# facebookresearch/FRL-Distributed-ML-Scaffold

Hardware: NVIDIA H100
Metric: samples/sec (whole box) on synthetic 2-task Problem (higher is better)
Workload: dtype bf16

## Files before the change

### frl-distributed-ml-scaffold_b200/_native.py

```python
import ctypes as C
import os
import subprocess
from typing import Optional, Sequence

import torch

_HERE = os.path.dirname(os.path.abspath(__file__))
CSRC_DIR = os.path.join(_HERE, "csrc")
LIB_PATH = os.path.join(CSRC_DIR, "libfrl_b200.so")

F32, BF16, U8, I64 = 0, 1, 2, 3
LOSS_MSE, LOSS_CE, LOSS_CE_PROB = 0, 1, 2
FP8_E4M3, FP8_E5M2 = 0, 1
FP8_DTYPE = {FP8_E4M3: torch.float8_e4m3fn, FP8_E5M2: torch.float8_e5m2}
MAX_TASKS = 8

_DTYPE_CODE = {torch.float32: F32, torch.bfloat16: BF16, torch.uint8: U8, torch.bool: U8,
               torch.int64: I64}


class NativeLibraryError(RuntimeError):
    pass


# ... 19 lines not shown
    "frl_launch_count": (C.c_uint64, []),
    "frl_launch_count_reset": (None, []),
    "frl_device_sm_count": (_i, []),
    "frl_device_arch": (_i, []),
    "frl_sgd_momentum": (_i, [_vp, _vp, _vp, _vp, _i64, _d, _d, _d, _d, _d, _vp, _vp, _i, _i, _vp]),
    "frl_adam": (_i, [_vp, _vp, _vp, _vp, _vp, _vp, _i64, _d, _d, _d, _d, _d, _i64, _d, _vp, _vp, _i, _vp]),
    "frl_rmsprop": (_i, [_vp, _vp, _vp, _vp, _vp, _i64, _d, _d, _d, _d, _d, _d, _vp, _vp, _i, _vp]),
    "frl_mt_tile_elems": (_i64, []),
    "frl_flatten_grads": (_i, [_vp, _vp, _vp, _i64, _vp, _i, _d, _vp]),
    "frl_sgd_momentum_mt": (_i, [_vp, _vp, _vp, _vp, _vp, _vp, _i64, _d, _d, _d, _d, _d, _vp, _vp, _i, _vp]),
    "frl_adam_mt": (_i, [_vp, _vp, _vp, _vp, _vp, _vp, _vp, _vp, _i64, _d, _d, _d, _d, _d, _i64, _d, _vp, _vp, _vp]),
    "frl_rmsprop_mt": (_i, [_vp, _vp, _vp, _vp, _vp, _vp, _vp, _i64, _d, _d, _d, _d, _d, _d, _vp, _vp, _vp]),
    "frl_layerwise_scratch_bytes": (_i64, [_i64, _i64]),
    "frl_lars_mt": (_i, [_vp, _vp, _vp, _vp, _vp, _vp, _i64, _i64, _vp, _vp, _vp, _d, _d, _d, _d, _vp, _vp, _i, _vp]),
    "frl_lamb_mt": (_i, [_vp, _vp, _vp, _vp, _vp, _vp, _vp, _i64, _i64, _vp, _vp, _vp, _d, _d, _d, _d, _d, _i64,
                         _d, _vp, _vp, _vp]),
    "frl_grad_accumulate_mt": (_i, [_vp, _vp, _vp, _vp, _i64, _d, _i, _vp, _vp]),
    "frl_weight_ema": (_i, [_vp, _vp, _i64, _d, _vp]),
    "frl_reduce_scratch_bytes": (_i64, []),
    "frl_grad_sumsq_clip": (_i, [_vp, _i64, _i, _f, _f, _vp, _vp, _vp]),
    "frl_criteria_scratch_bytes": (_i64, [_i]),
    "frl_criteria_forward": (_i, [C.POINTER(TaskDesc), _i, _vp, _vp, _vp, _vp, _vp, _vp, _vp]),
    "frl_criteria_backward": (_i, [C.POINTER(TaskDesc), _i, _vp, _vp, _vp, _vp]),
    "frl_preproc_affine": (_i, [_vp, _i, _vp, _i, _i64, _i64, _i64, _vp, _vp, _vp]),
    "frl_cast_scale": (_i, [_vp, _i, _vp, _i, _i64, _f, _vp]),
    "frl_augment_images": (_i, [_vp, _i64, _i, _i, _i, _vp, C.c_uint64, _i, _i, _d, _d, _d, _d, _d, _i, _i,
                                _vp, _vp, _vp, _i, _i, _i, _vp, _vp]),
    "frl_augment_mix_images": (_i, [_vp, _i64, _i, _i, _i, _vp, C.c_uint64, _i, _i, _d, _d, _d, _d, _d, _i, _i,
                                    _vp, _vp, _vp, _i, _i, _i, _vp, _i, _f, _i, _i, _i, _i, _vp]),
    "frl_mix_targets": (_i, [_vp, _i, _i64, _i64, _i, _f, _vp, _vp]),
    "frl_colsum_scratch_bytes": (_i64, [_i64, _i64]),
    "frl_colsum": (_i, [_vp, _i, _i64, _i64, _vp, _i, _i, _vp, _vp]),
    "frl_drelu_colsum": (_i, [_vp, _vp, _vp, _i, _i64, _i64, _vp, _i, _i, _vp, _vp]),
    "frl_gather_rows": (_i, [_vp, _i64, _vp, _vp, _i64, _i64, _i, _vp]),
    "frl_gather_rows_tma": (_i, [_vp, _i64, _vp, _vp, _i64, _i64, _i, _vp]),
    "frl_gather_window_rows": (_i, [_vp, _vp, _i, _vp, _vp, _i64, _i64, _vp]),
    "frl_gather_lines": (_i, [_vp, _i64, _i64, _vp, _i64, _vp, _vp, _i64, _i64, _i, _i, _vp]),
    "frl_gather_pool_create": (_vp, [_i]),
    "frl_gather_pool_destroy": (None, [_vp]),
    "frl_gather_pool_threads": (_i, [_vp]),
    "frl_gather_pool_submit": (_i64, [_vp, _vp, _i64, _vp, _vp, _i64, _i64]),
    "frl_gather_pool_submit_f32_to_bf16": (_i64, [_vp, _vp, _i64, _vp, _vp, _i64, _i64]),
    "frl_gather_pool_wait": (_i, [_vp, _i64]),
    "frl_nvls_sgd": (_i, [_vp, _vp, _vp, _vp, _i64, _i, _i, _vp, _i, _vp, _i, _d, _d, _d, _d, _d, _vp, _i, _i, _i, _vp]),
    "frl_nvls_adam": (_i, [_vp, _vp, _vp, _vp, _vp, _vp, _i64, _i, _i, _vp, _i, _vp, _i, _d, _d, _d, _d, _d,
                           _i64, _d, _vp, _i, _i, _vp]),
# ... 196 lines not shown

def criteria_scratch_bytes(n_tasks: int) -> int:
    return int(lib().frl_criteria_scratch_bytes(n_tasks))


def make_task_array(descs: Sequence[TaskDesc]):
    arr = (TaskDesc * len(descs))()
    for i, d in enumerate(descs):
        arr[i] = d
    return arr


def criteria_forward(task_array, n_tasks, losses, aux, lse, sink, nan_flag, scratch) -> None:
    _check(lib().frl_criteria_forward(task_array, n_tasks, _ptr(losses), _ptr(aux), _ptr(lse),
                                      _ptr(sink), _ptr(nan_flag), _ptr(scratch), _stream()),
           "frl_criteria_forward")


def criteria_backward(task_array, n_tasks, grad_losses, aux, lse) -> None:
    _check(lib().frl_criteria_backward(task_array, n_tasks, _ptr(grad_losses), _ptr(aux),
                                       _ptr(lse), _stream()), "frl_criteria_backward")



def preproc_affine(src, dst, *, inner=1, channels=1, scale=None, bias=None) -> None:
    n = src.numel()
    assert dst.numel() == n and src.is_contiguous() and dst.is_contiguous()
    _check(lib().frl_preproc_affine(_ptr(src), dtype_code(src.dtype), _ptr(dst),
                                    dtype_code(dst.dtype), n, inner, channels, _ptr(scale),
                                    _ptr(bias), _stream()), "frl_preproc_affine")


AUG_RRC, AUG_PAD_CROP, AUG_CENTER_RESIZE, AUG_CENTER_CROP = 0, 1, 2, 3


MIX_MIXUP, MIX_CUTMIX = 1, 2


def _augment_args(src, idx, dst, seed, epoch, mode, scale_range, ratio_range, eval_crop, pad, flip, scale, bias,
                  params_out):
    B, Cc, H, W = src.shape
    assert src.dtype == torch.uint8 and src.is_contiguous() and dst.is_contiguous()
    assert dst.dim() == 4 and tuple(dst.shape[:2]) == (B, Cc)
    assert idx.dtype == torch.int64 and idx.is_contiguous() and idx.numel() == B
    assert params_out is None or (params_out.dtype == torch.int32 and params_out.is_contiguous()
                                  and tuple(params_out.shape) == (B, 5))
# ... 219 lines not shown
```

### frl-distributed-ml-scaffold_b200/arena_linear.py

```python
import os
import types
from collections import Counter
from typing import List, Optional

import torch
import torch.nn as nn
import torch.nn.functional as F

from . import _native
from .types import Precision

KERNELS = _native

FP8_MULTIPLE = 16


def fp8_site_qualifies(uses_lp: bool, in_features: int, out_features: int) -> bool:
    return bool(uses_lp) and in_features % FP8_MULTIPLE == 0 and out_features % FP8_MULTIPLE == 0


def fp8_call_qualifies(x: torch.Tensor) -> bool:
    if x.dim() == 0 or x.shape[-1] == 0 or x.dtype not in (torch.bfloat16, torch.float32):
        return False
    m = x.numel() // x.shape[-1]
# ... 106 lines not shown
            y2 = saved[-1].reshape(-1, dz.shape[1])
            if in_step:
                dz_relu = torch.empty_like(dz)
                KERNELS.drelu_colsum(dz, y2, dz_relu, pipe.arena.grad_view(site.bslot),
                                     accumulate=not site.bstate.first_touch(pipe.step_id))
                dz, db_written = dz_relu, True
            else:
                dz = torch.ops.aten.threshold_backward(dz, y2, 0)
        need_dx = ctx.needs_input_grad[0]
        gemms = (_Fp8Gemms if ctx.fp8 else _DenseGemms)(saved, dz, need_dx)
        dx = gemms.dx().view(ctx.x_shape) if need_dx else None
        if in_step:
            site.weight_grad(pipe, gemms)
            if ctx.has_bias and not db_written and site.bslot is not None:
                KERNELS.colsum(dz.contiguous(), pipe.arena.grad_view(site.bslot),
                               accumulate=not site.bstate.first_touch(pipe.step_id))
            site.backward_done(pipe)
            return dx, None, None, None, None, None
        dw = gemms.dw(gemms.dzt) if ctx.needs_input_grad[1] else None
        db = dz.sum(0) if (ctx.has_bias and ctx.needs_input_grad[2]) else None
        return dx, dw, db, None, None, None


class _ArenaMultiHeadFn(torch.autograd.Function):

    @staticmethod
    def forward(ctx, x, site, *params):
        ctx.site = site
        ctx.save_for_backward(x)
        ctx.n_heads = len(params) // 2
        return tuple(F.linear(x, params[2 * i], params[2 * i + 1]) for i in range(ctx.n_heads))

    @staticmethod
    @torch.autograd.function.once_differentiable
    def backward(ctx, *dys):
        (x,) = ctx.saved_tensors
        site = ctx.site
        pipe = site.pipeline
        dy = torch.cat(dys, dim=1)
        dx = dy.matmul(site.weight_cat()) if ctx.needs_input_grad[0] else None
        none = (None,) * (2 * ctx.n_heads)
        if pipe is not None and pipe.step_open:
            gw = site.grad_weight_cat()
            if site.heads[0].wstate.first_touch(pipe.step_id):
                torch.mm(dy.t(), x, out=gw)
            else:
                gw.addmm_(dy.t(), x)
            for h in site.heads[1:]:
                h.wstate.first_touch(pipe.step_id)
            gb = site.grad_bias_cat()
            if gb is not None:
                first = site.heads[0].bstate.first_touch(pipe.step_id)
                for h in site.heads[1:]:
                    h.bstate.first_touch(pipe.step_id)
                KERNELS.colsum(dy, gb, accumulate=not first)
            else:
                for h, dyi in zip(site.heads, dys):
                    KERNELS.colsum(dyi.contiguous(), pipe.arena.grad_view(h.bslot),
                                   accumulate=not h.bstate.first_touch(pipe.step_id))
            for h in site.heads:
                h.backward_done(pipe)
            return (dx, None) + none
# ... 252 lines not shown
```

### frl-distributed-ml-scaffold_b200/criteria.py

```python
from abc import ABC, abstractmethod
from typing import Dict, List, Optional, Sequence, Tuple

import numpy as np
import torch
import torch.nn as nn
import torch.nn.functional as F
import torch.nn.modules.loss as L

from . import _native
from .types import LossType

KERNELS = _native



class MaskedLoss(L._Loss):

    def __init__(self, loss_layer, reduction: str = "mean") -> None:
        super().__init__(reduction=reduction)
        self.loss_layer = loss_layer

    def forward(self, *inputs) -> torch.Tensor:
        output, target, mask = inputs
        assert not target.requires_grad
# ... 160 lines not shown
    @staticmethod
    def forward(ctx, plan: _Plan, _unused, *outputs):
        outs = [o.contiguous() for o in outputs[:plan.n]]
        dev = outs[0].device
        losses = torch.empty(1 + plan.n, dtype=torch.float32, device=dev)
        aux = torch.empty(plan.n, dtype=torch.float32, device=dev)
        n_lse = sum(o.shape[0] * (2 if tp.kind == _native.LOSS_CE_PROB else 1)
                    for o, tp in zip(outs, plan.tasks) if tp.kind != _native.LOSS_MSE)
        lse = torch.empty(max(n_lse, 1), dtype=torch.float32, device=dev)
        arr, keep = _descs(plan, outs, None)
        KERNELS.criteria_forward(arr, plan.n, losses, aux, lse, plan.sink, plan.nan_flag,
                                 _scratch_for(dev, plan.n))
        ctx.plan = plan
        ctx.save_for_backward(aux, lse, *outs)
        ctx.set_materialize_grads(True)
        return losses

    @staticmethod
    @torch.autograd.function.once_differentiable
    def backward(ctx, grad_losses):
        plan = ctx.plan
        aux, lse, *outs = ctx.saved_tensors
        gl = grad_losses.contiguous().float()
        douts = [torch.empty_like(o) for o in outs]
        arr, keep = _descs(plan, outs, douts)
        KERNELS.criteria_backward(arr, plan.n, gl, aux, lse)
        return (None, None, *douts)


_path_logged = set()


def _log_path_once(modules, fused: bool) -> None:
    key = (tuple(type(m).__name__ for m in modules), fused)
    if key not in _path_logged:
        _path_logged.add(key)
        import logging
        logging.getLogger(__name__).info(
            "criterion path for loss modules %s: %s", list(key[0]),
            "fused kernels (frl_criteria_forward / _backward, one launch each)" if fused else
            "composed torch ops — outside the fused kernels' domain (MSE / CrossEntropy with mean "
            "reduction, optionally inside MaskedLoss; not class-weighted CrossEntropy or per-position "
            "probability targets)")


def fused_task_losses(modules, outputs, targets, weights=None, sink=None, nan_flag=None
                      ) -> Optional[torch.Tensor]:
    if not outputs or not outputs[0].is_cuda:
        return None
    plan = _plan_for(modules, outputs, targets, weights)
# ... 169 lines not shown
```

### frl-distributed-ml-scaffold_b200/csrc/criteria.cu

```cuda
#include "frl_common.cuh"

namespace frl {

constexpr int kCThreads = 256;
constexpr int kCWarps = kCThreads / 32;
constexpr int kCMaxBlocksPerTask = 528;
constexpr int kCVecPerLane = 8;
constexpr int kCRowChunk = 32 * 4 * kCVecPerLane;

struct CritParams {
    frl_task_desc t[FRL_MAX_TASKS];
    int nblk[FRL_MAX_TASKS];
    int blk_start[FRL_MAX_TASKS];
    int part_off[FRL_MAX_TASKS];
    int64_t lse_off[FRL_MAX_TASKS];
    int n_tasks;
    int total_blocks;
};

struct CritScratchHeader {
    unsigned int ticket;
    unsigned int _pad[3];
};
static inline int64_t crit_scratch_bytes(int T) {
    return static_cast<int64_t>(sizeof(CritScratchHeader)) +
           3ll * T * kCMaxBlocksPerTask * static_cast<int64_t>(sizeof(float));
}

template <typename T> __device__ __forceinline__ float ldf(const void* base, int64_t i);
template <> __device__ __forceinline__ float ldf<float>(const void* base, int64_t i) {
    return __ldg(static_cast<const float*>(base) + i);
}
template <> __device__ __forceinline__ float ldf<__nv_bfloat16>(const void* base, int64_t i) {
    return __bfloat162float(__ldg(static_cast<const __nv_bfloat16*>(base) + i));
}
__device__ __forceinline__ float ld_any(const void* base, int dtype, int64_t i) {
    return dtype == FRL_F32 ? ldf<float>(base, i) : ldf<__nv_bfloat16>(base, i);
}
// ... 18 lines not shown
    *reinterpret_cast<f32x4*>(static_cast<float*>(base) + e) = v;
}
template <> __device__ __forceinline__ void st4<__nv_bfloat16>(void* base, int64_t e, const f32x4& v) {
    *reinterpret_cast<bf16x4*>(static_cast<__nv_bfloat16*>(base) + e) =
        bf16x4{pack_bf16(v.x, v.y), pack_bf16(v.z, v.w)};
}

template <typename T> struct Raw4;
template <> struct Raw4<float> { f32x4 v; };
template <> struct Raw4<__nv_bfloat16> { bf16x4 v; };
__device__ __forceinline__ Raw4<float> ldraw4(const float* base, int64_t e) {
    return Raw4<float>{*reinterpret_cast<const f32x4*>(base + e)};
}
__device__ __forceinline__ Raw4<__nv_bfloat16> ldraw4(const __nv_bfloat16* base, int64_t e) {
    return Raw4<__nv_bfloat16>{*reinterpret_cast<const bf16x4*>(base + e)};
}
__device__ __forceinline__ f32x4 cvt4(const Raw4<float>& r) { return r.v; }
__device__ __forceinline__ f32x4 cvt4(const Raw4<__nv_bfloat16>& r) {
    return f32x4{bf16lo(r.v.a), bf16hi(r.v.a), bf16lo(r.v.b), bf16hi(r.v.b)};
}
__device__ __forceinline__ void fill_neg_inf(Raw4<float>& r) { r.v = f32x4{-INFINITY, -INFINITY, -INFINITY, -INFINITY}; }
__device__ __forceinline__ void fill_neg_inf(Raw4<__nv_bfloat16>& r) { r.v = bf16x4{0xff80ff80u, 0xff80ff80u}; }

__device__ __forceinline__ bool vec_ok(const frl_task_desc& t) {
    const int esz = t.out_dtype == FRL_F32 ? 4 : 2;
    return (t.cols % 4 == 0) && ((reinterpret_cast<uintptr_t>(t.out) % (4 * esz)) == 0) &&
           (t.dout == nullptr || (reinterpret_cast<uintptr_t>(t.dout) % (4 * esz)) == 0);
}

template <typename OT>
__device__ __forceinline__ void mse_partial(const frl_task_desc& t, int blk, int nblk,
                                            float& sum, float& nsel) {
    const int64_t n = t.rows * t.cols;
    const int64_t stride = static_cast<int64_t>(nblk) * kCThreads;
    float s = 0.f, c = 0.f;
    for (int64_t e = static_cast<int64_t>(blk) * kCThreads + threadIdx.x; e < n; e += stride) {
        if (t.mask && t.mask[e / t.mask_inner] == 0) continue;
        const float d = ldf<OT>(t.out, e) - ld_any(t.tgt, t.tgt_dtype, e);
        s = fmaf(d, d, s);
        c += 1.f;
    }
    sum = s;
    nsel = c;
}

__device__ __forceinline__ float soft_w(const frl_task_desc& t, bool prob, int64_t r0, int64_t c, int64_t y,
                                       float keep, float eps_c) {
    if (prob) return fmaf(keep, ld_any(t.tgt, t.tgt_dtype, r0 + c), eps_c);
    return (c == y ? keep : 0.f) + eps_c;
}

template <typename OT, bool SOFT>
__device__ __forceinline__ void ce_partial(const frl_task_desc& t, int blk, int nblk, float* lse_out,
                                           float& sum, float& nsel, float& nvalid) {
    const int lane = threadIdx.x & 31, warp = threadIdx.x >> 5;
    const int64_t C = t.cols;
    const bool vec = vec_ok(t);
    const int64_t* labels = static_cast<const int64_t*>(t.tgt);
    const bool prob = SOFT && t.kind == FRL_LOSS_CE_PROB;
// ... 20 lines not shown
                m = fmaxf(fmaxf(m, fmaxf(v.x, v.y)), fmaxf(v.z, v.w));
            }
            m = warp_max(m);
#pragma unroll
            for (int j = 0; j < kCVecPerLane; ++j) {
                if (lane * 4 + j * 128 < C) {
                    const f32x4 v = cvt4(q[j]);
                    has_nan |= (v.x != v.x) | (v.y != v.y) | (v.z != v.z) | (v.w != v.w);
                    se += expf(v.x - m) + expf(v.y - m) + expf(v.z - m) + expf(v.w - m);
                    if (soft) {
                        const int64_t c = lane * 4 + j * 128;
                        const float w0 = soft_w(t, prob, r0, c, ys, keep, eps_c);
                        const float w1 = soft_w(t, prob, r0, c + 1, ys, keep, eps_c);
                        const float w2 = soft_w(t, prob, r0, c + 2, ys, keep, eps_c);
                        const float w3 = soft_w(t, prob, r0, c + 3, ys, keep, eps_c);
                        aw += w0 * (m - v.x) + w1 * (m - v.y) + w2 * (m - v.z) + w3 * (m - v.w);
                        sw += (w0 + w1) + (w2 + w3);
                    }
                }
            }
        } else if (vec) {
            float mr = -INFINITY, sr = 0.f;
            for (int64_t cb = 0; cb < C; cb += kCRowChunk) {
                f32x4 v[kCVecPerLane];
#pragma unroll
                for (int j = 0; j < kCVecPerLane; ++j) {
                    const int64_t c = cb + lane * 4 + j * 128;
                    v[j] = c < C ? ld4<OT>(t.out, r0 + c) : f32x4{-INFINITY, -INFINITY, -INFINITY, -INFINITY};
                }
                float ml = -INFINITY;
#pragma unroll
                for (int j = 0; j < kCVecPerLane; ++j)
                    ml = fmaxf(fmaxf(ml, fmaxf(v[j].x, v[j].y)), fmaxf(v[j].z, v[j].w));
                const float mn = fmaxf(mr, ml);
                float add = 0.f;
                if (soft && mr != -INFINITY) aw = fmaf(sw, mn - mr, aw);
#pragma unroll
                for (int j = 0; j < kCVecPerLane; ++j) {
                    if (cb + lane * 4 + j * 128 < C) {
                        has_nan |= (v[j].x != v[j].x) | (v[j].y != v[j].y) | (v[j].z != v[j].z) | (v[j].w != v[j].w);
                        add += expf(v[j].x - mn) + expf(v[j].y - mn) + expf(v[j].z - mn) + expf(v[j].w - mn);
                        if (soft) {
                            const int64_t c = cb + lane * 4 + j * 128;
                            const float w0 = soft_w(t, prob, r0, c, ys, keep, eps_c);
                            const float w1 = soft_w(t, prob, r0, c + 1, ys, keep, eps_c);
                            const float w2 = soft_w(t, prob, r0, c + 2, ys, keep, eps_c);
                            const float w3 = soft_w(t, prob, r0, c + 3, ys, keep, eps_c);
                            aw += w0 * (mn - v[j].x) + w1 * (mn - v[j].y) + w2 * (mn - v[j].z) + w3 * (mn - v[j].w);
                            sw += (w0 + w1) + (w2 + w3);
                        }
                    }
                }
                sr = (mn == -INFINITY) ? 0.f : fmaf(sr, expf(mr - mn), add);
                mr = mn;
            }
            m = warp_max(mr);
            se = (mr == -INFINITY) ? 0.f : sr * expf(mr - m);
            if (soft && mr != -INFINITY) aw = fmaf(sw, m - mr, aw);

        } else {
            for (int64_t c = lane; c < C; c += 32) m = fmaxf(m, ldf<OT>(t.out, r0 + c));
            m = warp_max(m);
            for (int64_t c = lane; c < C; c += 32) {
                const float x = ldf<OT>(t.out, r0 + c);
                has_nan |= (x != x);
                se += expf(x - m);
                if (soft) {
                    const float w = soft_w(t, prob, r0, c, ys, keep, eps_c);
                    aw = fmaf(w, m - x, aw);
                    sw += w;
                }
// ... 22 lines not shown
                    s_sel += 1.f;
                    if (ys != static_cast<int64_t>(t.ignore_index)) {
                        s_valid += 1.f;
                        s_loss += (ys >= 0 && ys < C && !has_nan) ? fmaf(sw, logf(se), aw)
                                                                 : __int_as_float(0x7fc00000);
                    }
                }
            } else if (sel) {
                s_sel += 1.f;
                const int64_t y = labels[row];
                if (y != static_cast<int64_t>(t.ignore_index)) {
                    s_valid += 1.f;
                    s_loss += (y >= 0 && y < C) ? (lse - ldf<OT>(t.out, r0 + y))
                                                : __int_as_float(0x7fc00000);
                }
            }
        }
    }
    sum = s_loss;
    nsel = s_sel;
    nvalid = s_valid;
}

template <bool SOFT>
__global__ void __launch_bounds__(kCThreads, 5)
criteria_fwd_kernel(const __grid_constant__ CritParams P, float* __restrict__ losses,
                    float* __restrict__ aux, float* __restrict__ lse,
                    float* __restrict__ sink, int32_t* __restrict__ nan_flag,
                    CritScratchHeader* __restrict__ hdr) {
    __shared__ float smem[32];
    __shared__ bool is_last;
    int ti = 0;
#pragma unroll
    for (int i = 1; i < FRL_MAX_TASKS; ++i)
        if (i < P.n_tasks && static_cast<int>(blockIdx.x) >= P.blk_start[i]) ti = i;
    const int blk = static_cast<int>(blockIdx.x) - P.blk_start[ti];
    const frl_task_desc& t = P.t[ti];
    const int npart = P.n_tasks * kCMaxBlocksPerTask;
    float* part_sum = reinterpret_cast<float*>(hdr + 1);
    float* part_sel = part_sum + npart;
    float* part_valid = part_sel + npart;

    float s = 0.f, nsel = 0.f, nvalid = 0.f;
    if (t.kind == FRL_LOSS_MSE) {
        if (t.out_dtype == FRL_F32) mse_partial<float>(t, blk, P.nblk[ti], s, nsel);
        else                        mse_partial<__nv_bfloat16>(t, blk, P.nblk[ti], s, nsel);
        nvalid = nsel;
    } else {
        float* lse_t = lse + P.lse_off[ti];
        if (t.out_dtype == FRL_F32) ce_partial<float, SOFT>(t, blk, P.nblk[ti], lse_t, s, nsel, nvalid);
        else                        ce_partial<__nv_bfloat16, SOFT>(t, blk, P.nblk[ti], lse_t, s, nsel, nvalid);
    }
    s = block_sum(s, smem);
    nsel = block_sum(nsel, smem);
    nvalid = block_sum(nvalid, smem);
    if (threadIdx.x == 0) {
        const int slot = P.part_off[ti] + blk;
        part_sum[slot] = s;
        part_sel[slot] = nsel;
        part_valid[slot] = nvalid;
        __threadfence();
        is_last = (atomicAdd(&hdr->ticket, 1u) == static_cast<unsigned int>(P.total_blocks - 1));
    }
    __syncthreads();
    if (!is_last) return;
    __threadfence();

    __shared__ double dsm[kCWarps][3];
    const int lane = threadIdx.x & 31, warp = threadIdx.x >> 5;
    float total = 0.f;
    for (int i = 0; i < P.n_tasks; ++i) {
        double ds = 0.0, dsel = 0.0, dvalid = 0.0;
        for (int b = threadIdx.x; b < P.nblk[i]; b += kCThreads) {
            ds += static_cast<double>(__ldcg(part_sum + P.part_off[i] + b));
// ... 18 lines not shown
            if (q.mask != nullptr && dsel == 0.0) {
                if (q.kind == FRL_LOSS_MSE)     Li = 0.f;
                else if (SOFT && q.kind == FRL_LOSS_CE_PROB) Li = q.label_smoothing * logf(static_cast<float>(q.cols));
                else if (q.ignore_index == 0)   Li = __int_as_float(0x7fc00000);
                else                            Li = logf(static_cast<float>(q.cols));
            } else {
                Li = static_cast<float>(ds / dvalid);
            }
            Li *= q.weight;
            aux[i] = dvalid > 0.0 ? static_cast<float>(1.0 / dvalid) : 0.f;
            losses[1 + i] = Li;
            if (sink) sink[1 + i] = Li;
            total += Li;
        }
    }
    if (threadIdx.x == 0) {
        losses[0] = total;
        if (sink) sink[0] = total;
        if (nan_flag && (total != total)) *nan_flag = 1;
        hdr->ticket = 0;
    }
}

template <typename OT>
__device__ __forceinline__ void mse_bwd(const frl_task_desc& t, int blk, int nblk, float coef) {
    const int64_t n = t.rows * t.cols;
    const int64_t stride = static_cast<int64_t>(nblk) * kCThreads;
    for (int64_t e = static_cast<int64_t>(blk) * kCThreads + threadIdx.x; e < n; e += stride) {
        float d = 0.f;
        if (!(t.mask && t.mask[e / t.mask_inner] == 0))
            d = (ldf<OT>(t.out, e) - ld_any(t.tgt, t.tgt_dtype, e)) * coef;
        stf<OT>(t.dout, e, d);
    }
}

template <typename OT, bool SOFT>
__device__ __forceinline__ void ce_bwd(const frl_task_desc& t, int blk, int nblk, const float* lse,
                                       float coef) {
    const int lane = threadIdx.x & 31, warp = threadIdx.x >> 5;
    const int64_t C = t.cols;
    const bool vec = vec_ok(t);
    const int64_t* labels = static_cast<const int64_t*>(t.tgt);
    const bool prob = SOFT && t.kind == FRL_LOSS_CE_PROB;
    const bool soft = SOFT && (prob || t.label_smoothing != 0.f);
    const float keep = 1.f - t.label_smoothing, eps_c = t.label_smoothing / static_cast<float>(C);
    for (int64_t row = static_cast<int64_t>(blk) * kCWarps + warp; row < t.rows;
         row += static_cast<int64_t>(nblk) * kCWarps) {
        const int64_t r0 = row * C;
        const int64_t y = prob ? -1 : labels[row];
        const bool use = ((t.mask == nullptr) || (t.mask[row] != 0)) &&
                         (prob || y != static_cast<int64_t>(t.ignore_index));
        const float k = use ? coef : 0.f;
        const float l = lse[row];
        if (soft) {
            const float sq = prob ? lse[t.rows + row] : 1.f;
            if (vec) {
                for (int64_t cb = 0; cb < C; cb += kCRowChunk) {
                    f32x4 v[kCVecPerLane];
#pragma unroll
                    for (int j = 0; j < kCVecPerLane; ++j) {
                        const int64_t c = cb + lane * 4 + j * 128;
                        if (c < C) v[j] = ld4<OT>(t.out, r0 + c);
                    }
#pragma unroll
                    for (int j = 0; j < kCVecPerLane; ++j) {
                        const int64_t c = cb + lane * 4 + j * 128;
                        if (c >= C) break;
                        f32x4 q = v[j];
                        q.x = (expf(q.x - l) * sq - soft_w(t, prob, r0, c + 0, y, keep, eps_c)) * k;
                        q.y = (expf(q.y - l) * sq - soft_w(t, prob, r0, c + 1, y, keep, eps_c)) * k;
                        q.z = (expf(q.z - l) * sq - soft_w(t, prob, r0, c + 2, y, keep, eps_c)) * k;
                        q.w = (expf(q.w - l) * sq - soft_w(t, prob, r0, c + 3, y, keep, eps_c)) * k;
                        if (!use) q = f32x4{0.f, 0.f, 0.f, 0.f};
                        st4<OT>(t.dout, r0 + c, q);
                    }
                }
            } else {
                for (int64_t c = lane; c < C; c += 32) {
                    const float x = ldf<OT>(t.out, r0 + c);
                    stf<OT>(t.dout, r0 + c,
                            use ? (expf(x - l) * sq - soft_w(t, prob, r0, c, y, keep, eps_c)) * k : 0.f);
                }
            }
        } else if (vec) {
            for (int64_t cb = 0; cb < C; cb += kCRowChunk) {
                f32x4 v[kCVecPerLane];
#pragma unroll
                for (int j = 0; j < kCVecPerLane; ++j) {
                    const int64_t c = cb + lane * 4 + j * 128;
                    if (c < C) v[j] = ld4<OT>(t.out, r0 + c);
                }
#pragma unroll
                for (int j = 0; j < kCVecPerLane; ++j) {
                    const int64_t c = cb + lane * 4 + j * 128;
                    if (c >= C) break;
                    f32x4 q = v[j];
                    q.x = (expf(q.x - l) - (c + 0 == y ? 1.f : 0.f)) * k;
                    q.y = (expf(q.y - l) - (c + 1 == y ? 1.f : 0.f)) * k;
                    q.z = (expf(q.z - l) - (c + 2 == y ? 1.f : 0.f)) * k;
                    q.w = (expf(q.w - l) - (c + 3 == y ? 1.f : 0.f)) * k;
                    if (!use) q = f32x4{0.f, 0.f, 0.f, 0.f};
                    st4<OT>(t.dout, r0 + c, q);
                }
            }
        } else {
            for (int64_t c = lane; c < C; c += 32) {
                const float x = ldf<OT>(t.out, r0 + c);
                stf<OT>(t.dout, r0 + c, use ? (expf(x - l) - (c == y ? 1.f : 0.f)) * k : 0.f);
            }
        }
    }
}

template <bool SOFT>
__global__ void __launch_bounds__(kCThreads, 5)
criteria_bwd_kernel(const __grid_constant__ CritParams P, const float* __restrict__ gl,
                    const float* __restrict__ aux, const float* __restrict__ lse) {
    int ti = 0;
#pragma unroll
    for (int i = 1; i < FRL_MAX_TASKS; ++i)
        if (i < P.n_tasks && static_cast<int>(blockIdx.x) >= P.blk_start[i]) ti = i;
    const int blk = static_cast<int>(blockIdx.x) - P.blk_start[ti];
    const frl_task_desc& t = P.t[ti];
    const float scale = (__ldg(gl) + __ldg(gl + 1 + ti)) * t.weight * __ldg(aux + ti);
    if (t.kind == FRL_LOSS_MSE) {
        const float coef = 2.f * scale;
        if (t.out_dtype == FRL_F32) mse_bwd<float>(t, blk, P.nblk[ti], coef);
        else                        mse_bwd<__nv_bfloat16>(t, blk, P.nblk[ti], coef);
    } else {
        const float* lse_t = lse + P.lse_off[ti];
        if (t.out_dtype == FRL_F32) ce_bwd<float, SOFT>(t, blk, P.nblk[ti], lse_t, scale);
        else                        ce_bwd<__nv_bfloat16, SOFT>(t, blk, P.nblk[ti], lse_t, scale);
    }
}

static int build_params(const frl_task_desc* tasks, int T, bool backward, CritParams& P, int& max_blk,
                        bool& soft, const char* name) {
    FRL_REQUIRE(tasks != nullptr && T >= 1, FRL_E_ARG, "%s: no tasks", name);
    FRL_REQUIRE(T <= FRL_MAX_TASKS, FRL_E_TOO_MANY, "%s: at most %d tasks", name, FRL_MAX_TASKS);
    int off = 0;
    int64_t lse_off = 0;
    max_blk = 1;
    soft = false;
    P.n_tasks = T;
    for (int i = 0; i < T; ++i) {
        const frl_task_desc& t = tasks[i];
        FRL_REQUIRE(t.kind == FRL_LOSS_MSE || t.kind == FRL_LOSS_CE || t.kind == FRL_LOSS_CE_PROB, FRL_E_ARG,
                    "%s: task %d kind", name, i);
        FRL_REQUIRE(t.label_smoothing >= 0.f && t.label_smoothing <= 1.f, FRL_E_ARG,
                    "%s: task %d label_smoothing must be in [0, 1], got %g", name, i, t.label_smoothing);
        FRL_REQUIRE(t.kind != FRL_LOSS_MSE || t.label_smoothing == 0.f, FRL_E_ARG,
                    "%s: task %d label_smoothing on an MSE task", name, i);
        FRL_REQUIRE(t.out_dtype == FRL_F32 || t.out_dtype == FRL_BF16, FRL_E_DTYPE, "%s: task %d out dtype", name, i);
        FRL_REQUIRE(t.rows >= 0 && t.cols >= 1, FRL_E_ARG, "%s: task %d shape", name, i);
        FRL_REQUIRE(t.rows == 0 || (t.out && t.tgt), FRL_E_ARG, "%s: task %d null out/tgt", name, i);
        FRL_REQUIRE(!backward || t.rows == 0 || t.dout, FRL_E_ARG, "%s: task %d null dout", name, i);
        if (t.kind == FRL_LOSS_MSE) {
            FRL_REQUIRE(t.tgt_dtype == FRL_F32 || t.tgt_dtype == FRL_BF16, FRL_E_DTYPE, "%s: task %d tgt dtype", name, i);
            FRL_REQUIRE(!t.mask || t.mask_inner >= 1, FRL_E_ARG, "%s: task %d mask_inner", name, i);
        } else if (t.kind == FRL_LOSS_CE_PROB) {
            FRL_REQUIRE(t.tgt_dtype == FRL_F32 || t.tgt_dtype == FRL_BF16, FRL_E_DTYPE,
                        "%s: task %d CE probability targets must be FRL_F32 or FRL_BF16", name, i);
            FRL_REQUIRE(!t.mask || t.mask_inner == t.cols, FRL_E_ARG, "%s: task %d CE mask is per row", name, i);
        } else {
            FRL_REQUIRE(t.tgt_dtype == FRL_I64, FRL_E_DTYPE, "%s: task %d CE labels must be int64", name, i);
            FRL_REQUIRE(!t.mask || t.mask_inner == t.cols, FRL_E_ARG, "%s: task %d CE mask is per row", name, i);
        }
        soft |= t.kind == FRL_LOSS_CE_PROB || t.label_smoothing != 0.f;
        P.t[i] = t;
        int64_t work_blocks;
        if (t.kind == FRL_LOSS_MSE) work_blocks = (t.rows * t.cols + kCThreads * 8 - 1) / (kCThreads * 8);
        else                        work_blocks = (t.rows + kCWarps - 1) / kCWarps;
        if (work_blocks < 1) work_blocks = 1;
        if (work_blocks > kCMaxBlocksPerTask) work_blocks = kCMaxBlocksPerTask;
        P.nblk[i] = static_cast<int>(work_blocks);
        P.part_off[i] = off;
        off += kCMaxBlocksPerTask;
        P.lse_off[i] = lse_off;
        if (t.kind == FRL_LOSS_CE) lse_off += t.rows;
        if (t.kind == FRL_LOSS_CE_PROB) lse_off += 2 * t.rows;
        if (P.nblk[i] > max_blk) max_blk = P.nblk[i];
    }
    int total = 0;
    for (int i = 0; i < T; ++i) {
        P.blk_start[i] = total;
        total += P.nblk[i];
    }
    P.total_blocks = total;
    return 0;
}

}

using namespace frl;

extern "C" int64_t frl_criteria_scratch_bytes(int n_tasks) {
    if (n_tasks < 1 || n_tasks > FRL_MAX_TASKS) return -1;
    return crit_scratch_bytes(n_tasks);
}

extern "C" int frl_criteria_forward(const frl_task_desc* tasks_host, int n_tasks, float* losses,
                                    float* aux, float* lse, float* sink_mapped,
                                    int32_t* nan_flag_mapped, void* scratch, void* stream) {
    CritParams P;
    int max_blk = 1;
    bool soft = false;
    const int rc = build_params(tasks_host, n_tasks, false, P, max_blk, soft, "frl_criteria_forward");
    if (rc) return rc;
    FRL_REQUIRE(losses && aux && scratch, FRL_E_ARG, "frl_criteria_forward: null outputs");
    bool any_ce = false;
    for (int i = 0; i < n_tasks; ++i) any_ce |= (tasks_host[i].kind != FRL_LOSS_MSE);
    FRL_REQUIRE(!any_ce || lse, FRL_E_ARG, "frl_criteria_forward: CE task needs lse buffer");
    const int grid = P.total_blocks;
    cudaStream_t st = static_cast<cudaStream_t>(stream);
    CritScratchHeader* hdr = static_cast<CritScratchHeader*>(scratch);
    if (soft) criteria_fwd_kernel<true><<<grid, kCThreads, 0, st>>>(P, losses, aux, lse, sink_mapped, nan_flag_mapped, hdr);
    else      criteria_fwd_kernel<false><<<grid, kCThreads, 0, st>>>(P, losses, aux, lse, sink_mapped, nan_flag_mapped, hdr);
    return after_launch("frl_criteria_forward");
}

extern "C" int frl_criteria_backward(const frl_task_desc* tasks_host, int n_tasks,
                                     const float* grad_losses, const float* aux, const float* lse,
                                     void* stream) {
    CritParams P;
    int max_blk = 1;
    bool soft = false;
    const int rc = build_params(tasks_host, n_tasks, true, P, max_blk, soft, "frl_criteria_backward");
    if (rc) return rc;
    FRL_REQUIRE(grad_losses && aux, FRL_E_ARG, "frl_criteria_backward: null inputs");
    const int grid = P.total_blocks;
    cudaStream_t st = static_cast<cudaStream_t>(stream);
    if (soft) criteria_bwd_kernel<true><<<grid, kCThreads, 0, st>>>(P, grad_losses, aux, lse);
    else      criteria_bwd_kernel<false><<<grid, kCThreads, 0, st>>>(P, grad_losses, aux, lse);
    return after_launch("frl_criteria_backward");
}
```

### include/frl_b200.h

```cpp
#ifndef FRL_B200_H
#define FRL_B200_H

#include <stdint.h>

#ifdef __cplusplus
extern "C" {
#endif

#define FRL_ABI_VERSION 1

enum { FRL_F32 = 0, FRL_BF16 = 1, FRL_U8 = 2, FRL_I64 = 3 };
enum { FRL_E_ARG = -1, FRL_E_ALIGN = -2, FRL_E_DTYPE = -3, FRL_E_TOO_MANY = -4 };

int          frl_abi_version(void);
const char*  frl_last_error(void);
uint64_t     frl_launch_count(void);
void         frl_launch_count_reset(void);
int          frl_device_sm_count(void);
int          frl_device_arch(void);


int frl_sgd_momentum(float* p, const void* g, float* buf, void* p_lp, int64_t n,
                     double lr, double mu, double dampening, double wd,
                     double grad_scale, const float* grad_scale_dev, const float* dyn,
// ... 70 lines not shown
    int32_t     tgt_dtype;
    int32_t     ignore_index;
    const void* out;
    const void* tgt;
    const uint8_t* mask;
    void*       dout;
    int64_t     rows;
    int64_t     cols;
    int64_t     mask_inner;
    float       weight;
    float       label_smoothing;
} frl_task_desc;

int64_t frl_criteria_scratch_bytes(int n_tasks);

int frl_criteria_forward(const frl_task_desc* tasks_host, int n_tasks,
                         float* losses, float* aux, float* lse,
                         float* sink_mapped, int32_t* nan_flag_mapped,
                         void* scratch, void* stream);

int frl_criteria_backward(const frl_task_desc* tasks_host, int n_tasks,
                          const float* grad_losses, const float* aux, const float* lse,
                          void* stream);

int frl_preproc_affine(const void* src, int src_dtype, void* dst, int dst_dtype, int64_t n,
                       int64_t inner, int64_t channels, const float* scale, const float* bias,
                       void* stream);

enum { FRL_AUG_RRC = 0, FRL_AUG_PAD_CROP = 1, FRL_AUG_CENTER_RESIZE = 2, FRL_AUG_CENTER_CROP = 3 };
int frl_augment_images(const void* src, int64_t batch, int channels, int height, int width,
                       const int64_t* idx, uint64_t seed, int epoch, int mode,
                       double smin, double smax, double rmin, double rmax, double eval_crop, int pad,
                       int flip, const float* scale, const float* bias, void* dst, int dst_dtype,
                       int out_h, int out_w, int32_t* params_out, void* stream);

enum { FRL_MIX_MIXUP = 1, FRL_MIX_CUTMIX = 2 };
int frl_augment_mix_images(const void* src, int64_t batch, int channels, int height, int width,
                           const int64_t* idx, uint64_t seed, int epoch, int mode,
                           double smin, double smax, double rmin, double rmax, double eval_crop, int pad,
                           int flip, const float* scale, const float* bias, void* dst, int dst_dtype,
                           int out_h, int out_w, int32_t* params_out, int mix_mode, float lam,
                           int box_y0, int box_y1, int box_x0, int box_x1, void* stream);
int frl_mix_targets(const void* src, int src_dtype, int64_t batch, int64_t inner, int n_classes, float lam,
                    void* dst, void* stream);

int frl_cast_scale(const void* src, int src_dtype, void* dst, int dst_dtype, int64_t n,
// ... 58 lines not shown
```

Baseline: 1.925 million.

## Write multi-task loss grads into one packed buffer to skip head concat

The criteria backward now writes each task's output gradient into adjacent column slices of a single packed buffer through a new row-stride-aware entry point. The multi-head linear backward detects that the head gradients are adjacent views and uses them directly instead of calling torch.cat. The kernels are also specialised on a common output dtype, batch MSE loads eight deep for memory-level parallelism, and load bf16 raw before converting. The intent is to remove a concat copy and some per-element branching, at the cost of strided stores and more template instantiations.

```diff
diff --git a/frl-distributed-ml-scaffold_b200/_native.py b/frl-distributed-ml-scaffold_b200/_native.py
--- a/frl-distributed-ml-scaffold_b200/_native.py
+++ b/frl-distributed-ml-scaffold_b200/_native.py
@@ -65,6 +65,7 @@
     "frl_criteria_scratch_bytes": (_i64, [_i]),
     "frl_criteria_forward": (_i, [C.POINTER(TaskDesc), _i, _vp, _vp, _vp, _vp, _vp, _vp, _vp]),
     "frl_criteria_backward": (_i, [C.POINTER(TaskDesc), _i, _vp, _vp, _vp, _vp]),
+    "frl_criteria_backward_ld": (_i, [C.POINTER(TaskDesc), _i, _vp, _vp, _vp, C.POINTER(C.c_int64), _vp]),
     "frl_preproc_affine": (_i, [_vp, _i, _vp, _i, _i64, _i64, _i64, _vp, _vp, _vp]),
     "frl_cast_scale": (_i, [_vp, _i, _vp, _i, _i64, _f, _vp]),
     "frl_augment_images": (_i, [_vp, _i64, _i, _i, _i, _vp, C.c_uint64, _i, _i, _d, _d, _d, _d, _d, _i, _i,
@@ -307,6 +308,12 @@
                                        _ptr(lse), _stream()), "frl_criteria_backward")
 
 
+def criteria_backward_ld(task_array, n_tasks, grad_losses, aux, lse, row_strides) -> None:
+    ld = (C.c_int64 * n_tasks)(*row_strides)
+    _check(lib().frl_criteria_backward_ld(task_array, n_tasks, _ptr(grad_losses), _ptr(aux),
+                                          _ptr(lse), ld, _stream()), "frl_criteria_backward_ld")
+
+
 
 def preproc_affine(src, dst, *, inner=1, channels=1, scale=None, bias=None) -> None:
     n = src.numel()
diff --git a/frl-distributed-ml-scaffold_b200/arena_linear.py b/frl-distributed-ml-scaffold_b200/arena_linear.py
--- a/frl-distributed-ml-scaffold_b200/arena_linear.py
+++ b/frl-distributed-ml-scaffold_b200/arena_linear.py
@@ -152,6 +152,20 @@
         return dx, dw, db, None, None, None
 
 
+def _adjacent_columns(dys) -> Optional[torch.Tensor]:
+    d0 = dys[0]
+    if any(d is None or d.dim() != 2 for d in dys):
+        return None
+    rows, width = d0.shape[0], sum(d.shape[1] for d in dys)
+    ptr, off = d0.untyped_storage().data_ptr(), d0.storage_offset()
+    for d in dys:
+        if (d.dtype != d0.dtype or d.device != d0.device or d.shape[0] != rows or d.stride() != (width, 1)
+                or d.untyped_storage().data_ptr() != ptr or d.storage_offset() != off):
+            return None
+        off += d.shape[1]
+    return d0.as_strided((rows, width), (width, 1))
+
+
 class _ArenaMultiHeadFn(torch.autograd.Function):
 
     @staticmethod
@@ -167,7 +181,9 @@
         (x,) = ctx.saved_tensors
         site = ctx.site
         pipe = site.pipeline
-        dy = torch.cat(dys, dim=1)
+        dy = _adjacent_columns(dys)
+        if dy is None:
+            dy = torch.cat(dys, dim=1)
         dx = dy.matmul(site.weight_cat()) if ctx.needs_input_grad[0] else None
         none = (None,) * (2 * ctx.n_heads)
         if pipe is not None and pipe.step_open:
diff --git a/frl-distributed-ml-scaffold_b200/criteria.py b/frl-distributed-ml-scaffold_b200/criteria.py
--- a/frl-distributed-ml-scaffold_b200/criteria.py
+++ b/frl-distributed-ml-scaffold_b200/criteria.py
@@ -206,10 +206,23 @@
         plan = ctx.plan
         aux, lse, *outs = ctx.saved_tensors
         gl = grad_losses.contiguous().float()
-        douts = [torch.empty_like(o) for o in outs]
-        arr, keep = _descs(plan, outs, douts)
-        KERNELS.criteria_backward(arr, plan.n, gl, aux, lse)
+        if _packable(outs):
+            buf = torch.empty(outs[0].shape[0], sum(o.shape[1] for o in outs), dtype=outs[0].dtype,
+                              device=outs[0].device)
+            douts = list(buf.split([o.shape[1] for o in outs], dim=1))
+            arr, keep = _descs(plan, outs, douts)
+            KERNELS.criteria_backward_ld(arr, plan.n, gl, aux, lse, [buf.shape[1]] * plan.n)
+        else:
+            douts = [torch.empty_like(o) for o in outs]
+            arr, keep = _descs(plan, outs, douts)
+            KERNELS.criteria_backward(arr, plan.n, gl, aux, lse)
         return (None, None, *douts)
+
+
+def _packable(outs: Sequence[torch.Tensor]) -> bool:
+    o0 = outs[0]
+    return len(outs) > 1 and all(o.dim() == 2 and o.shape[0] == o0.shape[0] and o.dtype == o0.dtype
+                                 for o in outs)
 
 
 _path_logged = set()
diff --git a/frl-distributed-ml-scaffold_b200/csrc/criteria.cu b/frl-distributed-ml-scaffold_b200/csrc/criteria.cu
--- a/frl-distributed-ml-scaffold_b200/csrc/criteria.cu
+++ b/frl-distributed-ml-scaffold_b200/csrc/criteria.cu
@@ -1,3 +1,5 @@
+#include <type_traits>
+
 #include "frl_common.cuh"
 
 namespace frl {
@@ -14,6 +16,7 @@
     int blk_start[FRL_MAX_TASKS];
     int part_off[FRL_MAX_TASKS];
     int64_t lse_off[FRL_MAX_TASKS];
+    int64_t dld[FRL_MAX_TASKS];
     int n_tasks;
     int total_blocks;
 };
@@ -78,11 +81,17 @@
 __device__ __forceinline__ void fill_neg_inf(Raw4<float>& r) { r.v = f32x4{-INFINITY, -INFINITY, -INFINITY, -INFINITY}; }
 __device__ __forceinline__ void fill_neg_inf(Raw4<__nv_bfloat16>& r) { r.v = bf16x4{0xff80ff80u, 0xff80ff80u}; }
 
+template <typename OTF> __device__ __forceinline__ bool out_is_f32(int dtype) {
+    return std::is_same<OTF, float>::value || (std::is_same<OTF, void>::value && dtype == FRL_F32);
+}
+
 __device__ __forceinline__ bool vec_ok(const frl_task_desc& t) {
     const int esz = t.out_dtype == FRL_F32 ? 4 : 2;
     return (t.cols % 4 == 0) && ((reinterpret_cast<uintptr_t>(t.out) % (4 * esz)) == 0) &&
            (t.dout == nullptr || (reinterpret_cast<uintptr_t>(t.dout) % (4 * esz)) == 0);
 }
+
+constexpr int kMseBatch = 8;
 
 template <typename OT>
 __device__ __forceinline__ void mse_partial(const frl_task_desc& t, int blk, int nblk,
@@ -90,7 +99,26 @@
     const int64_t n = t.rows * t.cols;
     const int64_t stride = static_cast<int64_t>(nblk) * kCThreads;
     float s = 0.f, c = 0.f;
-    for (int64_t e = static_cast<int64_t>(blk) * kCThreads + threadIdx.x; e < n; e += stride) {
+    int64_t e = static_cast<int64_t>(blk) * kCThreads + threadIdx.x;
+    for (; e + (kMseBatch - 1) * stride < n; e += kMseBatch * stride) {
+        float o[kMseBatch], g[kMseBatch];
+        bool sel[kMseBatch];
+#pragma unroll
+        for (int u = 0; u < kMseBatch; ++u) {
+            const int64_t i = e + u * stride;
+            sel[u] = !(t.mask && t.mask[i / t.mask_inner] == 0);
+            o[u] = ldf<OT>(t.out, i);
+            g[u] = ld_any(t.tgt, t.tgt_dtype, i);
+        }
+#pragma unroll
+        for (int u = 0; u < kMseBatch; ++u) {
+            if (!sel[u]) continue;
+            const float d = o[u] - g[u];
+            s = fmaf(d, d, s);
+            c += 1.f;
+        }
+    }
+    for (; e < n; e += stride) {
         if (t.mask && t.mask[e / t.mask_inner] == 0) continue;
         const float d = ldf<OT>(t.out, e) - ld_any(t.tgt, t.tgt_dtype, e);
         s = fmaf(d, d, s);
@@ -157,31 +185,34 @@
         } else if (vec) {
             float mr = -INFINITY, sr = 0.f;
             for (int64_t cb = 0; cb < C; cb += kCRowChunk) {
-                f32x4 v[kCVecPerLane];
+                Raw4<OT> q[kCVecPerLane];
 #pragma unroll
                 for (int j = 0; j < kCVecPerLane; ++j) {
                     const int64_t c = cb + lane * 4 + j * 128;
-                    v[j] = c < C ? ld4<OT>(t.out, r0 + c) : f32x4{-INFINITY, -INFINITY, -INFINITY, -INFINITY};
+                    if (c < C) q[j] = ldraw4(static_cast<const OT*>(t.out), r0 + c); else fill_neg_inf(q[j]);
                 }
                 float ml = -INFINITY;
 #pragma unroll
-                for (int j = 0; j < kCVecPerLane; ++j)
-                    ml = fmaxf(fmaxf(ml, fmaxf(v[j].x, v[j].y)), fmaxf(v[j].z, v[j].w));
+                for (int j = 0; j < kCVecPerLane; ++j) {
+                    const f32x4 v = cvt4(q[j]);
+                    ml = fmaxf(fmaxf(ml, fmaxf(v.x, v.y)), fmaxf(v.z, v.w));
+                }
                 const float mn = fmaxf(mr, ml);
                 float add = 0.f;
                 if (soft && mr != -INFINITY) aw = fmaf(sw, mn - mr, aw);
 #pragma unroll
                 for (int j = 0; j < kCVecPerLane; ++j) {
                     if (cb + lane * 4 + j * 128 < C) {
-                        has_nan |= (v[j].x != v[j].x) | (v[j].y != v[j].y) | (v[j].z != v[j].z) | (v[j].w != v[j].w);
-                        add += expf(v[j].x - mn) + expf(v[j].y - mn) + expf(v[j].z - mn) + expf(v[j].w - mn);
+                        const f32x4 v = cvt4(q[j]);
+                        has_nan |= (v.x != v.x) | (v.y != v.y) | (v.z != v.z) | (v.w != v.w);
+                        add += expf(v.x - mn) + expf(v.y - mn) + expf(v.z - mn) + expf(v.w - mn);
                         if (soft) {
                             const int64_t c = cb + lane * 4 + j * 128;
                             const float w0 = soft_w(t, prob, r0, c, ys, keep, eps_c);
                             const float w1 = soft_w(t, prob, r0, c + 1, ys, keep, eps_c);
                             const float w2 = soft_w(t, prob, r0, c + 2, ys, keep, eps_c);
                             const float w3 = soft_w(t, prob, r0, c + 3, ys, keep, eps_c);
-                            aw += w0 * (mn - v[j].x) + w1 * (mn - v[j].y) + w2 * (mn - v[j].z) + w3 * (mn - v[j].w);
+                            aw += w0 * (mn - v.x) + w1 * (mn - v.y) + w2 * (mn - v.z) + w3 * (mn - v.w);
                             sw += (w0 + w1) + (w2 + w3);
                         }
                     }
@@ -250,7 +281,7 @@
     nvalid = s_valid;
 }
 
-template <bool SOFT>
+template <bool SOFT, typename OTF>
 __global__ void __launch_bounds__(kCThreads, 5)
 criteria_fwd_kernel(const __grid_constant__ CritParams P, float* __restrict__ losses,
                     float* __restrict__ aux, float* __restrict__ lse,
@@ -271,13 +302,13 @@
 
     float s = 0.f, nsel = 0.f, nvalid = 0.f;
     if (t.kind == FRL_LOSS_MSE) {
-        if (t.out_dtype == FRL_F32) mse_partial<float>(t, blk, P.nblk[ti], s, nsel);
-        else                        mse_partial<__nv_bfloat16>(t, blk, P.nblk[ti], s, nsel);
+        if (out_is_f32<OTF>(t.out_dtype)) mse_partial<float>(t, blk, P.nblk[ti], s, nsel);
+        else                              mse_partial<__nv_bfloat16>(t, blk, P.nblk[ti], s, nsel);
         nvalid = nsel;
     } else {
         float* lse_t = lse + P.lse_off[ti];
-        if (t.out_dtype == FRL_F32) ce_partial<float, SOFT>(t, blk, P.nblk[ti], lse_t, s, nsel, nvalid);
-        else                        ce_partial<__nv_bfloat16, SOFT>(t, blk, P.nblk[ti], lse_t, s, nsel, nvalid);
+        if (out_is_f32<OTF>(t.out_dtype)) ce_partial<float, SOFT>(t, blk, P.nblk[ti], lse_t, s, nsel, nvalid);
+        else                              ce_partial<__nv_bfloat16, SOFT>(t, blk, P.nblk[ti], lse_t, s, nsel, nvalid);
     }
     s = block_sum(s, smem);
     nsel = block_sum(nsel, smem);
@@ -342,31 +373,50 @@
     }
 }
 
+__device__ __forceinline__ int64_t dout_index(int64_t e, int64_t cols, int64_t ld) {
+    return ld == cols ? e : (e / cols) * ld + e % cols;
+}
+
 template <typename OT>
-__device__ __forceinline__ void mse_bwd(const frl_task_desc& t, int blk, int nblk, float coef) {
+__device__ __forceinline__ void mse_bwd(const frl_task_desc& t, int blk, int nblk, float coef, int64_t ld) {
     const int64_t n = t.rows * t.cols;
     const int64_t stride = static_cast<int64_t>(nblk) * kCThreads;
-    for (int64_t e = static_cast<int64_t>(blk) * kCThreads + threadIdx.x; e < n; e += stride) {
+    int64_t e = static_cast<int64_t>(blk) * kCThreads + threadIdx.x;
+    for (; e + (kMseBatch - 1) * stride < n; e += kMseBatch * stride) {
+        float o[kMseBatch], g[kMseBatch];
+        bool sel[kMseBatch];
+#pragma unroll
+        for (int u = 0; u < kMseBatch; ++u) {
+            const int64_t i = e + u * stride;
+            sel[u] = !(t.mask && t.mask[i / t.mask_inner] == 0);
+            o[u] = ldf<OT>(t.out, i);
+            g[u] = ld_any(t.tgt, t.tgt_dtype, i);
+        }
+#pragma unroll
+        for (int u = 0; u < kMseBatch; ++u)
+            stf<OT>(t.dout, dout_index(e + u * stride, t.cols, ld), sel[u] ? (o[u] - g[u]) * coef : 0.f);
+    }
+    for (; e < n; e += stride) {
         float d = 0.f;
         if (!(t.mask && t.mask[e / t.mask_inner] == 0))
             d = (ldf<OT>(t.out, e) - ld_any(t.tgt, t.tgt_dtype, e)) * coef;
-        stf<OT>(t.dout, e, d);
+        stf<OT>(t.dout, dout_index(e, t.cols, ld), d);
     }
 }
 
 template <typename OT, bool SOFT>
 __device__ __forceinline__ void ce_bwd(const frl_task_desc& t, int blk, int nblk, const float* lse,
-                                       float coef) {
+                                       float coef, int64_t ld) {
     const int lane = threadIdx.x & 31, warp = threadIdx.x >> 5;
     const int64_t C = t.cols;
-    const bool vec = vec_ok(t);
+    const bool vec = vec_ok(t) && (ld % 4 == 0);
     const int64_t* labels = static_cast<const int64_t*>(t.tgt);
     const bool prob = SOFT && t.kind == FRL_LOSS_CE_PROB;
     const bool soft = SOFT && (prob || t.label_smoothing != 0.f);
     const float keep = 1.f - t.label_smoothing, eps_c = t.label_smoothing / static_cast<float>(C);
     for (int64_t row = static_cast<int64_t>(blk) * kCWarps + warp; row < t.rows;
          row += static_cast<int64_t>(nblk) * kCWarps) {
-        const int64_t r0 = row * C;
+        const int64_t r0 = row * C, d0 = row * ld;
         const int64_t y = prob ? -1 : labels[row];
         const bool use = ((t.mask == nullptr) || (t.mask[row] != 0)) &&
                          (prob || y != static_cast<int64_t>(t.ignore_index));
@@ -376,63 +426,63 @@
             const float sq = prob ? lse[t.rows + row] : 1.f;
             if (vec) {
                 for (int64_t cb = 0; cb < C; cb += kCRowChunk) {
-                    f32x4 v[kCVecPerLane];
+                    Raw4<OT> v[kCVecPerLane];
 #pragma unroll
                     for (int j = 0; j < kCVecPerLane; ++j) {
                         const int64_t c = cb + lane * 4 + j * 128;
-                        if (c < C) v[j] = ld4<OT>(t.out, r0 + c);
+                        if (c < C) v[j] = ldraw4(static_cast<const OT*>(t.out), r0 + c);
                     }
 #pragma unroll
                     for (int j = 0; j < kCVecPerLane; ++j) {
                         const int64_t c = cb + lane * 4 + j * 128;
                         if (c >= C) break;
-                        f32x4 q = v[j];
+                        f32x4 q = cvt4(v[j]);
                         q.x = (expf(q.x - l) * sq - soft_w(t, prob, r0, c + 0, y, keep, eps_c)) * k;
                         q.y = (expf(q.y - l) * sq - soft_w(t, prob, r0, c + 1, y, keep, eps_c)) * k;
                         q.z = (expf(q.z - l) * sq - soft_w(t, prob, r0, c + 2, y, keep, eps_c)) * k;
                         q.w = (expf(q.w - l) * sq - soft_w(t, prob, r0, c + 3, y, keep, eps_c)) * k;
                         if (!use) q = f32x4{0.f, 0.f, 0.f, 0.f};
-                        st4<OT>(t.dout, r0 + c, q);
+                        st4<OT>(t.dout, d0 + c, q);
                     }
                 }
             } else {
                 for (int64_t c = lane; c < C; c += 32) {
                     const float x = ldf<OT>(t.out, r0 + c);
-                    stf<OT>(t.dout, r0 + c,
+                    stf<OT>(t.dout, d0 + c,
                             use ? (expf(x - l) * sq - soft_w(t, prob, r0, c, y, keep, eps_c)) * k : 0.f);
                 }
             }
         } else if (vec) {
             for (int64_t cb = 0; cb < C; cb += kCRowChunk) {
-                f32x4 v[kCVecPerLane];
+                Raw4<OT> v[kCVecPerLane];
 #pragma unroll
                 for (int j = 0; j < kCVecPerLane; ++j) {
                     const int64_t c = cb + lane * 4 + j * 128;
-                    if (c < C) v[j] = ld4<OT>(t.out, r0 + c);
+                    if (c < C) v[j] = ldraw4(static_cast<const OT*>(t.out), r0 + c);
                 }
 #pragma unroll
                 for (int j = 0; j < kCVecPerLane; ++j) {
                     const int64_t c = cb + lane * 4 + j * 128;
                     if (c >= C) break;
-                    f32x4 q = v[j];
+                    f32x4 q = cvt4(v[j]);
                     q.x = (expf(q.x - l) - (c + 0 == y ? 1.f : 0.f)) * k;
                     q.y = (expf(q.y - l) - (c + 1 == y ? 1.f : 0.f)) * k;
                     q.z = (expf(q.z - l) - (c + 2 == y ? 1.f : 0.f)) * k;
                     q.w = (expf(q.w - l) - (c + 3 == y ? 1.f : 0.f)) * k;
                     if (!use) q = f32x4{0.f, 0.f, 0.f, 0.f};
-                    st4<OT>(t.dout, r0 + c, q);
+                    st4<OT>(t.dout, d0 + c, q);
                 }
             }
         } else {
             for (int64_t c = lane; c < C; c += 32) {
                 const float x = ldf<OT>(t.out, r0 + c);
-                stf<OT>(t.dout, r0 + c, use ? (expf(x - l) - (c == y ? 1.f : 0.f)) * k : 0.f);
-            }
-        }
-    }
-}
-
-template <bool SOFT>
+                stf<OT>(t.dout, d0 + c, use ? (expf(x - l) - (c == y ? 1.f : 0.f)) * k : 0.f);
+            }
+        }
+    }
+}
+
+template <bool SOFT, typename OTF>
 __global__ void __launch_bounds__(kCThreads, 5)
 criteria_bwd_kernel(const __grid_constant__ CritParams P, const float* __restrict__ gl,
                     const float* __restrict__ aux, const float* __restrict__ lse) {
@@ -445,17 +495,17 @@
     const float scale = (__ldg(gl) + __ldg(gl + 1 + ti)) * t.weight * __ldg(aux + ti);
     if (t.kind == FRL_LOSS_MSE) {
         const float coef = 2.f * scale;
-        if (t.out_dtype == FRL_F32) mse_bwd<float>(t, blk, P.nblk[ti], coef);
-        else                        mse_bwd<__nv_bfloat16>(t, blk, P.nblk[ti], coef);
+        if (out_is_f32<OTF>(t.out_dtype)) mse_bwd<float>(t, blk, P.nblk[ti], coef, P.dld[ti]);
+        else                              mse_bwd<__nv_bfloat16>(t, blk, P.nblk[ti], coef, P.dld[ti]);
     } else {
         const float* lse_t = lse + P.lse_off[ti];
-        if (t.out_dtype == FRL_F32) ce_bwd<float, SOFT>(t, blk, P.nblk[ti], lse_t, scale);
-        else                        ce_bwd<__nv_bfloat16, SOFT>(t, blk, P.nblk[ti], lse_t, scale);
+        if (out_is_f32<OTF>(t.out_dtype)) ce_bwd<float, SOFT>(t, blk, P.nblk[ti], lse_t, scale, P.dld[ti]);
+        else                              ce_bwd<__nv_bfloat16, SOFT>(t, blk, P.nblk[ti], lse_t, scale, P.dld[ti]);
     }
 }
 
 static int build_params(const frl_task_desc* tasks, int T, bool backward, CritParams& P, int& max_blk,
-                        bool& soft, const char* name) {
+                        bool& soft, const char* name, const int64_t* dout_ld = nullptr) {
     FRL_REQUIRE(tasks != nullptr && T >= 1, FRL_E_ARG, "%s: no tasks", name);
     FRL_REQUIRE(T <= FRL_MAX_TASKS, FRL_E_TOO_MANY, "%s: at most %d tasks", name, FRL_MAX_TASKS);
     int off = 0;
@@ -488,6 +538,12 @@
         }
         soft |= t.kind == FRL_LOSS_CE_PROB || t.label_smoothing != 0.f;
         P.t[i] = t;
+        P.dld[i] = t.cols;
+        if (dout_ld != nullptr && dout_ld[i] != 0) {
+            FRL_REQUIRE(dout_ld[i] >= t.cols, FRL_E_ARG, "%s: task %d row stride %lld < cols %lld", name, i,
+                        static_cast<long long>(dout_ld[i]), static_cast<long long>(t.cols));
+            P.dld[i] = dout_ld[i];
+        }
         int64_t work_blocks;
         if (t.kind == FRL_LOSS_MSE) work_blocks = (t.rows * t.cols + kCThreads * 8 - 1) / (kCThreads * 8);
         else                        work_blocks = (t.rows + kCWarps - 1) / kCWarps;
@@ -509,6 +565,26 @@
     P.total_blocks = total;
     return 0;
 }
+
+static int common_out_dtype(const CritParams& P) {
+    for (int i = 1; i < P.n_tasks; ++i)
+        if (P.t[i].out_dtype != P.t[0].out_dtype) return -1;
+    return P.t[0].out_dtype;
+}
+
+#define FRL_CRIT_DISPATCH(LAUNCH)                                                                  \
+    do {                                                                                           \
+        const int dt = common_out_dtype(P);                                                        \
+        if (soft) {                                                                                \
+            if (dt == FRL_BF16) LAUNCH(true, __nv_bfloat16);                                       \
+            else if (dt == FRL_F32) LAUNCH(true, float);                                           \
+            else LAUNCH(true, void);                                                               \
+        } else {                                                                                   \
+            if (dt == FRL_BF16) LAUNCH(false, __nv_bfloat16);                                      \
+            else if (dt == FRL_F32) LAUNCH(false, float);                                          \
+            else LAUNCH(false, void);                                                              \
+        }                                                                                          \
+    } while (0)
 
 }
 
@@ -534,23 +610,39 @@
     const int grid = P.total_blocks;
     cudaStream_t st = static_cast<cudaStream_t>(stream);
     CritScratchHeader* hdr = static_cast<CritScratchHeader*>(scratch);
-    if (soft) criteria_fwd_kernel<true><<<grid, kCThreads, 0, st>>>(P, losses, aux, lse, sink_mapped, nan_flag_mapped, hdr);
-    else      criteria_fwd_kernel<false><<<grid, kCThreads, 0, st>>>(P, losses, aux, lse, sink_mapped, nan_flag_mapped, hdr);
+#define FRL_FWD(S, D) criteria_fwd_kernel<S, D><<<grid, kCThreads, 0, st>>>(P, losses, aux, lse, sink_mapped, nan_flag_mapped, hdr)
+    FRL_CRIT_DISPATCH(FRL_FWD);
+#undef FRL_FWD
     return after_launch("frl_criteria_forward");
+}
+
+static int criteria_backward(const frl_task_desc* tasks_host, int n_tasks, const float* grad_losses,
+                             const float* aux, const float* lse, const int64_t* dout_ld, void* stream,
+                             const char* name) {
+    CritParams P;
+    int max_blk = 1;
+    bool soft = false;
+    const int rc = build_params(tasks_host, n_tasks, true, P, max_blk, soft, name, dout_ld);
+    if (rc) return rc;
+    FRL_REQUIRE(grad_losses && aux, FRL_E_ARG, "%s: null inputs", name);
+    const int grid = P.total_blocks;
+    cudaStream_t st = static_cast<cudaStream_t>(stream);
+#define FRL_BWD(S, D) criteria_bwd_kernel<S, D><<<grid, kCThreads, 0, st>>>(P, grad_losses, aux, lse)
+    FRL_CRIT_DISPATCH(FRL_BWD);
+#undef FRL_BWD
+    return after_launch(name);
 }
 
 extern "C" int frl_criteria_backward(const frl_task_desc* tasks_host, int n_tasks,
                                      const float* grad_losses, const float* aux, const float* lse,
                                      void* stream) {
-    CritParams P;
-    int max_blk = 1;
-    bool soft = false;
-    const int rc = build_params(tasks_host, n_tasks, true, P, max_blk, soft, "frl_criteria_backward");
-    if (rc) return rc;
-    FRL_REQUIRE(grad_losses && aux, FRL_E_ARG, "frl_criteria_backward: null inputs");
-    const int grid = P.total_blocks;
-    cudaStream_t st = static_cast<cudaStream_t>(stream);
-    if (soft) criteria_bwd_kernel<true><<<grid, kCThreads, 0, st>>>(P, grad_losses, aux, lse);
-    else      criteria_bwd_kernel<false><<<grid, kCThreads, 0, st>>>(P, grad_losses, aux, lse);
-    return after_launch("frl_criteria_backward");
-}
+    return criteria_backward(tasks_host, n_tasks, grad_losses, aux, lse, nullptr, stream,
+                             "frl_criteria_backward");
+}
+
+extern "C" int frl_criteria_backward_ld(const frl_task_desc* tasks_host, int n_tasks,
+                                        const float* grad_losses, const float* aux, const float* lse,
+                                        const int64_t* dout_ld, void* stream) {
+    return criteria_backward(tasks_host, n_tasks, grad_losses, aux, lse, dout_ld, stream,
+                             "frl_criteria_backward_ld");
+}
diff --git a/include/frl_b200.h b/include/frl_b200.h
--- a/include/frl_b200.h
+++ b/include/frl_b200.h
@@ -116,6 +116,10 @@
 int frl_criteria_backward(const frl_task_desc* tasks_host, int n_tasks,
                           const float* grad_losses, const float* aux, const float* lse,
                           void* stream);
+
+int frl_criteria_backward_ld(const frl_task_desc* tasks_host, int n_tasks,
+                             const float* grad_losses, const float* aux, const float* lse,
+                             const int64_t* dout_ld, void* stream);
 
 int frl_preproc_affine(const void* src, int src_dtype, void* dst, int dst_dtype, int64_t n,
                        int64_t inner, int64_t channels, const float* scale, const float* bias,
```

Result: no change. 1.940 million (median of 6 runs) (+0.8%).
